# Iamctb/ImageStitching

Hardware: AMD Instinct MI355X
Metric: stitched megapixels/sec (9x12 MP vertical) (higher is better)
Workload: dtype u8

## Files before the change

### imagestitching_amd/csrc/ist_host.cpp

```cpp
#include "ist_host.h"

#include <algorithm>
#include <atomic>
#include <cstring>
#include <mutex>
#include <string>
#include <thread>

#include "ist_internal.h"

namespace ist {

namespace {

constexpr size_t kPoolGranule = 2u << 20;
constexpr size_t kPoolKeepBytes = 2ull << 30;
constexpr size_t kPoolKeepBlocks = 6;

constexpr size_t kPoolKeepBatchBytes = 8ull << 30;
constexpr size_t kPoolKeepBatchBlocks = 256;

struct Block { void* p; size_t cap; bool busy; uint64_t stamp; bool batch = false; };
std::mutex g_pool_mu;
std::vector<Block>& pool() { static std::vector<Block>* v = new std::vector<Block>(); return *v; }
uint64_t g_pool_clock = 0;

void pool_enforce_class_locked(bool batch) {
  const size_t keep_bytes = batch ? kPoolKeepBatchBytes : kPoolKeepBytes, keep_blocks = batch ? kPoolKeepBatchBlocks : kPoolKeepBlocks;
  for (;;) {
    size_t idle_bytes = 0, idle = 0, oldest = SIZE_MAX;
    std::vector<Block>& v = pool();
    for (size_t i = 0; i < v.size(); ++i) {
      if (v[i].busy || v[i].batch != batch) continue;
      idle_bytes += v[i].cap; ++idle;
      if (oldest == SIZE_MAX || v[i].stamp < v[oldest].stamp) oldest = i;
    }
    if (oldest == SIZE_MAX || (idle_bytes <= keep_bytes && idle <= keep_blocks)) return;
    (void)hipHostFree(v[oldest].p);
    v.erase(v.begin() + static_cast<std::ptrdiff_t>(oldest));
  }
}

void* pool_take_class(size_t bytes, bool batch) {
  const size_t need = ((bytes ? bytes : 1) + kPoolGranule - 1) / kPoolGranule * kPoolGranule;
  {
    std::lock_guard<std::mutex> lock(g_pool_mu);
    std::vector<Block>& v = pool();
    size_t best = SIZE_MAX;
    for (size_t i = 0; i < v.size(); ++i)
      if (!v[i].busy && v[i].batch == batch && v[i].cap >= need && v[i].cap <= 2 * need && (best == SIZE_MAX || v[i].cap < v[best].cap)) best = i;
    if (best != SIZE_MAX) { v[best].busy = true; v[best].stamp = ++g_pool_clock; return v[best].p; }
  }
  void* p = nullptr;
  if (hipHostMalloc(&p, need, hipHostMallocPortable) != hipSuccess) {
    (void)hipGetLastError();
    pool_trim();
    if (hipHostMalloc(&p, need, hipHostMallocPortable) != hipSuccess) { (void)hipGetLastError(); return nullptr; }
  }
  std::lock_guard<std::mutex> lock(g_pool_mu);
  pool().push_back(Block{p, need, true, ++g_pool_clock, batch});
  return p;
}

}

void* pool_take(size_t bytes) { return pool_take_class(bytes, false); }
void* pool_take_batch(size_t bytes) { return pool_take_class(bytes, true); }

bool pool_give(void* p) {
  std::lock_guard<std::mutex> lock(g_pool_mu);
  for (Block& b : pool())
    if (b.p == p) {
      b.busy = false; b.stamp = ++g_pool_clock;
      pool_enforce_class_locked(b.batch);
      return true;
    }
  return false;
}

void pool_trim() {
  std::lock_guard<std::mutex> lock(g_pool_mu);
  std::vector<Block>& v = pool();
  for (size_t i = v.size(); i-- > 0;)
    if (!v[i].busy) { (void)hipHostFree(v[i].p); v.erase(v.begin() + static_cast<std::ptrdiff_t>(i)); }
}

namespace {

constexpr size_t kChunk = 4u << 20;
constexpr int kLanes = 4;

struct Piece { uint32_t item; size_t row0, n_rows, col0, n_cols; };

void split(const std::vector<RowsCopy>& items, std::vector<Piece>* out) {
  for (size_t k = 0; k < items.size(); ++k) {
    const RowsCopy& it = items[k];
    if (it.row == 0 || it.rows == 0) continue;
    if (it.row <= kChunk) {
      const size_t per = kChunk / it.row;
      for (size_t r = 0; r < it.rows; r += per) out->push_back(Piece{static_cast<uint32_t>(k), r, std::min(per, it.rows - r), 0, it.row});
    } else {
      for (size_t r = 0; r < it.rows; ++r)
        for (size_t c = 0; c < it.row; c += kChunk) out->push_back(Piece{static_cast<uint32_t>(k), r, 1, c, std::min(kChunk, it.row - c)});
    }
  }
}

inline size_t piece_bytes(const Piece& p) { return p.n_rows * p.n_cols; }

void pack(const RowsCopy& it, const Piece& p, uint8_t* chunk) {
  const uint8_t* s = static_cast<const uint8_t*>(it.host_src) + p.row0 * it.host_pitch + p.col0;
  if (it.host_pitch == p.n_cols) { std::memcpy(chunk, s, p.n_rows * p.n_cols); return; }
  for (size_t r = 0; r < p.n_rows; ++r) std::memcpy(chunk + r * p.n_cols, s + r * it.host_pitch, p.n_cols);
}
void unpack(const RowsCopy& it, const Piece& p, const uint8_t* chunk) {
  uint8_t* d = static_cast<uint8_t*>(it.host_dst) + p.row0 * it.host_pitch + p.col0;
  if (it.host_pitch == p.n_cols) { std::memcpy(d, chunk, p.n_rows * p.n_cols); return; }
  for (size_t r = 0; r < p.n_rows; ++r) std::memcpy(d + r * it.host_pitch, chunk + r * p.n_cols, p.n_cols);
}
inline uint8_t* dev_of(const RowsCopy& it, const Piece& p) { return static_cast<uint8_t*>(it.dev) + p.row0 * it.row + p.col0; }

}

void Stager::release_lane(Lane& l) {
  if (l.stream) (void)hipStreamSynchronize(l.stream);
  for (int s = 0; s < 2; ++s) { if (l.done[s]) (void)hipEventDestroy(l.done[s]); if (l.chunk[s]) (void)hipHostFree(l.chunk[s]); l.done[s] = nullptr; l.chunk[s] = nullptr; }
  if (l.tail) (void)hipEventDestroy(l.tail);
  if (l.stream) (void)hipStreamDestroy(l.stream);
  l.tail = nullptr; l.stream = nullptr;
}

Stager::~Stager() {
  int prev = -1;
  (void)hipGetDevice(&prev);
  if (hipSetDevice(device_) != hipSuccess) return;
  if (big_.stream) (void)hipStreamSynchronize(big_.stream);
  for (int s = 0; s < 2; ++s) { if (big_.done[s]) (void)hipEventDestroy(big_.done[s]); if (big_.piece[s]) (void)hipHostFree(big_.piece[s]); }
  if (big_.tail) (void)hipEventDestroy(big_.tail);
  if (big_.stream) (void)hipStreamDestroy(big_.stream);
  for (Lane& l : lanes_) release_lane(l);
  if (gate_) (void)hipEventDestroy(gate_);
  if (prev >= 0) (void)hipSetDevice(prev);
}

int Stager::ensure() {
  if (!lanes_.empty()) return IST_OK;
  std::vector<Lane> lanes(kLanes);
  hipEvent_t gate = nullptr;
  bool ok = hipEventCreateWithFlags(&gate, hipEventDisableTiming) == hipSuccess;
  for (Lane& l : lanes) {
    ok = ok && hipStreamCreateWithFlags(&l.stream, hipStreamNonBlocking) == hipSuccess &&
         hipEventCreateWithFlags(&l.tail, hipEventDisableTiming) == hipSuccess;
    for (int s = 0; s < 2 && ok; ++s)
      ok = hipHostMalloc(&l.chunk[s], kChunk, hipHostMallocDefault) == hipSuccess &&
           hipEventCreateWithFlags(&l.done[s], hipEventDisableTiming) == hipSuccess &&
           hipEventRecord(l.done[s], l.stream) == hipSuccess;
  }
  if (!ok) {
    (void)hipGetLastError();
    for (Lane& l : lanes) release_lane(l);
    if (gate) (void)hipEventDestroy(gate);
    return fail(IST_E_HIP, "allocating the pinned staging ring failed");
  }
  lanes_.swap(lanes);
  gate_ = gate;
  return IST_OK;
}

namespace { constexpr size_t kBigPiece = 32u << 20; constexpr int kBigPackers = 4; }

int Stager::ensure_big() {
  if (big_.stream) return IST_OK;
  Big b;
  bool ok = hipStreamCreateWithFlags(&b.stream, hipStreamNonBlocking) == hipSuccess && hipEventCreateWithFlags(&b.tail, hipEventDisableTiming) == hipSuccess;
  for (int s = 0; s < 2 && ok; ++s)
    ok = hipHostMalloc(&b.piece[s], kBigPiece, hipHostMallocDefault) == hipSuccess && hipEventCreateWithFlags(&b.done[s], hipEventDisableTiming) == hipSuccess &&
         hipEventRecord(b.done[s], b.stream) == hipSuccess;
  if (!ok) {
    (void)hipGetLastError();
    for (int s = 0; s < 2; ++s) { if (b.done[s]) (void)hipEventDestroy(b.done[s]); if (b.piece[s]) (void)hipHostFree(b.piece[s]); }
    if (b.tail) (void)hipEventDestroy(b.tail);
    if (b.stream) (void)hipStreamDestroy(b.stream);
    return fail(IST_E_HIP, "allocating the large staging pieces failed");
  }
  big_ = b;
  return IST_OK;
}

int Stager::upload_big(const std::vector<RowsCopy>& items, hipStream_t after, WorkerPool* pool) {
  if (!pool) return upload(items, after);
  std::vector<RowsCopy> small;
  bool any = false;
  for (const RowsCopy& it : items) { if (it.row == 0 || it.rows == 0) continue; if (it.row > kBigPiece) small.push_back(it); else any = true; }
  if (!small.empty()) { const int rc = upload(small, after); if (rc) return rc; }
  if (!any) return IST_OK;
  int rc = ensure_big();
  if (rc) return rc;
  for (const RowsCopy& it : items) {
    if (it.row == 0 || it.rows == 0 || it.row > kBigPiece) continue;
    if (it.host_pitch == it.row) {
      hipPointerAttribute_t attr;
      std::memset(&attr, 0, sizeof(attr));
      if (hipPointerGetAttributes(&attr, it.host_src) == hipSuccess && attr.type == hipMemoryTypeHost) {
        if (hipMemcpyAsync(it.dev, it.host_src, it.rows * it.row, hipMemcpyHostToDevice, big_.stream) != hipSuccess) { (void)hipGetLastError(); return fail(IST_E_HIP, "host-to-device copy failed"); }
        continue;
      }
      (void)hipGetLastError();
    }
    const size_t per = std::max<size_t>(1, kBigPiece / it.row);
    for (size_t r0 = 0; r0 < it.rows; r0 += per) {
      const size_t nr = std::min(per, it.rows - r0);
      const int s = static_cast<int>(big_.k++ & 1u);
      if (hipEventSynchronize(big_.done[s]) != hipSuccess) { (void)hipGetLastError(); return fail(IST_E_HIP, "host-to-device staging failed"); }
      uint8_t* piece = static_cast<uint8_t*>(big_.piece[s]);
      const int workers = static_cast<int>(std::min<size_t>(kBigPackers, std::max<size_t>(1, nr * it.row >> 20)));
      const size_t share = (nr + static_cast<size_t>(workers) - 1) / static_cast<size_t>(workers);
      auto part = [&](int w) {
        const size_t a = static_cast<size_t>(w) * share, b = std::min(nr, a + share);
        if (a >= b) return;
        const uint8_t* src = static_cast<const uint8_t*>(it.host_src) + (r0 + a) * it.host_pitch;
        if (it.host_pitch == it.row) std::memcpy(piece + a * it.row, src, (b - a) * it.row);
        else for (size_t r = a; r < b; ++r) std::memcpy(piece + r * it.row, src + (r - a) * it.host_pitch, it.row);
      };
      if (workers > 1) { pool->run(workers, part); pool->wait(); } else part(0);
      if (hipMemcpyAsync(static_cast<uint8_t*>(it.dev) + r0 * it.row, piece, nr * it.row, hipMemcpyHostToDevice, big_.stream) != hipSuccess ||
          hipEventRecord(big_.done[s], big_.stream) != hipSuccess) { (void)hipGetLastError(); return fail(IST_E_HIP, "host-to-device staging failed"); }
    }
  }
  if (hipEventRecord(big_.tail, big_.stream) != hipSuccess || hipStreamWaitEvent(after, big_.tail, 0) != hipSuccess) { (void)hipGetLastError(); return fail(IST_E_HIP, "ordering the uploads before the launch failed"); }
  return IST_OK;
}

int Stager::sync() {
  bool ok = true;
  if (big_.stream) ok = hipStreamSynchronize(big_.stream) == hipSuccess;
  for (Lane& l : lanes_) if (l.stream) ok = (hipStreamSynchronize(l.stream) == hipSuccess) && ok;
  return ok ? IST_OK : fail(IST_E_HIP, "hipStreamSynchronize failed");
}

int Stager::upload(const std::vector<RowsCopy>& items, hipStream_t after) { return run(items, true, after); }
int Stager::download(const std::vector<RowsCopy>& items, hipStream_t before) { return run(items, false, before); }

int Stager::run(const std::vector<RowsCopy>& items, bool up, hipStream_t other) {
  std::vector<Piece> pieces;
  split(items, &pieces);
  if (pieces.empty()) return IST_OK;
  int rc = ensure();
  if (rc) return rc;
  size_t total = 0;
  for (const Piece& p : pieces) total += piece_bytes(p);
  const int n_lanes = total < (2u << 20) ? 1 : static_cast<int>(std::min<size_t>(kLanes, pieces.size()));
  if (!up) {
    if (hipEventRecord(gate_, other) != hipSuccess) return fail(IST_E_HIP, "hipEventRecord failed");
    for (int l = 0; l < n_lanes; ++l)
      if (hipStreamWaitEvent(lanes_[static_cast<size_t>(l)].stream, gate_, 0) != hipSuccess) return fail(IST_E_HIP, "hipStreamWaitEvent failed");
  }
  std::atomic<size_t> next{0};
  std::atomic<int> err{0};
  auto work = [&](int li) {
    if (hipSetDevice(device_) != hipSuccess) { err = 1; return; }
    Lane& L = lanes_[static_cast<size_t>(li)];
    const Piece* pending[2] = {nullptr, nullptr};
    unsigned k = 0;
    for (;;) {
      const size_t i = next.fetch_add(1);
      if (i >= pieces.size() || err.load()) break;
      const Piece& p = pieces[i];
      const RowsCopy& it = items[p.item];
      const int s = static_cast<int>(k++ & 1u);
      if (hipEventSynchronize(L.done[s]) != hipSuccess) { err = 1; break; }
      uint8_t* chunk = static_cast<uint8_t*>(L.chunk[s]);
      if (up) {
        pack(it, p, chunk);
        if (hipMemcpyAsync(dev_of(it, p), chunk, piece_bytes(p), hipMemcpyHostToDevice, L.stream) != hipSuccess) { err = 1; break; }
      } else {
        if (pending[s]) { unpack(items[pending[s]->item], *pending[s], chunk); pending[s] = nullptr; }
        if (hipMemcpyAsync(chunk, dev_of(it, p), piece_bytes(p), hipMemcpyDeviceToHost, L.stream) != hipSuccess) { err = 1; break; }
        pending[s] = &p;
      }
      if (hipEventRecord(L.done[s], L.stream) != hipSuccess) { err = 1; break; }
    }
    if (!up)
      for (unsigned d = 0; d < 2; ++d) {
        const int s = static_cast<int>((k + d) & 1u);
        if (!pending[s]) continue;
        if (hipEventSynchronize(L.done[s]) != hipSuccess) { err = 1; continue; }
        unpack(items[pending[s]->item], *pending[s], static_cast<const uint8_t*>(L.chunk[s]));
      }
  };
  if (n_lanes == 1) work(0);
  else {
    std::vector<std::thread> th;
    for (int l = 1; l < n_lanes; ++l) th.emplace_back(work, l);
    work(0);
    for (std::thread& t : th) t.join();
  }
  if (err.load()) { (void)hipGetLastError(); return fail(IST_E_HIP, up ? "host-to-device staging failed" : "device-to-host staging failed"); }
  if (up)
    for (int l = 0; l < n_lanes; ++l) {
      Lane& L = lanes_[static_cast<size_t>(l)];
      if (hipEventRecord(L.tail, L.stream) != hipSuccess || hipStreamWaitEvent(other, L.tail, 0) != hipSuccess)
        return fail(IST_E_HIP, "ordering the uploads before the launch failed");
    }
  return IST_OK;
}


WorkerPool::~WorkerPool() {
  { std::lock_guard<std::mutex> lock(mu_); stop_ = true; }
  work_cv_.notify_all();
  for (std::thread& t : th_) if (t.joinable()) t.join();
}

void WorkerPool::loop() {
  std::unique_lock<std::mutex> lock(mu_);
  for (;;) {
    work_cv_.wait(lock, [&]() { return stop_ || next_ < total_; });
    if (stop_) return;
    const int i = next_++;
    lock.unlock();
    fn_(i);
    lock.lock();
    if (++done_ == total_) done_cv_.notify_all();
  }
}

void WorkerPool::run(int n, std::function<void(int)> fn) {
  if (n <= 0) return;
  {
    std::lock_guard<std::mutex> lock(mu_);
    tl_mark("pool: queue locked");
    fn_ = std::move(fn);
    next_ = 0; done_ = 0; total_ = n;
    const size_t want = static_cast<size_t>(n < kMaxThreads ? n : kMaxThreads);
    while (th_.size() < want) th_.emplace_back([this]() { loop(); });
  }
  tl_mark("pool: tasks posted");
  work_cv_.notify_all();
  tl_mark("pool: workers notified");
}

void WorkerPool::wait() {
  std::unique_lock<std::mutex> lock(mu_);
  done_cv_.wait(lock, [&]() { return done_ == total_; });
  total_ = 0; next_ = 0; done_ = 0;
}

}
```

### imagestitching_amd/csrc/ist_host.h

```cpp
#ifndef IST_HOST_H_
#define IST_HOST_H_

#include <hip/hip_runtime_api.h>

#include <cstddef>
#include <thread>
#include <mutex>
#include <functional>
#include <condition_variable>
#include <cstdint>
#include <vector>

#include "ist_internal.h"

namespace ist {

void* pool_take(size_t bytes);
void* pool_take_batch(size_t bytes);
bool pool_give(void* p);
void pool_trim();

class Stager {
 public:
  explicit Stager(int device) : device_(device) {}
  ~Stager();
  Stager(const Stager&) = delete;
  Stager& operator=(const Stager&) = delete;
  int upload(const std::vector<RowsCopy>& items, hipStream_t after);
  int download(const std::vector<RowsCopy>& items, hipStream_t before);
  int sync();
  int upload_big(const std::vector<RowsCopy>& items, hipStream_t after, class WorkerPool* pool);

 private:
  struct Lane { hipStream_t stream = nullptr; void* chunk[2] = {nullptr, nullptr}; hipEvent_t done[2] = {nullptr, nullptr}; hipEvent_t tail = nullptr; };
  int ensure();
  static void release_lane(Lane& l);
  int run(const std::vector<RowsCopy>& items, bool up, hipStream_t other);
  int device_;
  std::vector<Lane> lanes_;
  hipEvent_t gate_ = nullptr;
  struct Big { hipStream_t stream = nullptr; void* piece[2] = {nullptr, nullptr}; hipEvent_t done[2] = {nullptr, nullptr}; hipEvent_t tail = nullptr; unsigned k = 0; } big_;
  int ensure_big();
};


class WorkerPool {
 public:
  static constexpr int kMaxThreads = 32;
  WorkerPool() = default;
  ~WorkerPool();
  WorkerPool(const WorkerPool&) = delete;
  WorkerPool& operator=(const WorkerPool&) = delete;
  void run(int n, std::function<void(int)> fn);
  void wait();
 private:
  void loop();
  std::mutex mu_;
  std::condition_variable work_cv_, done_cv_;
  std::vector<std::thread> th_;
  std::function<void(int)> fn_;
  int next_ = 0, total_ = 0, done_ = 0;
  bool stop_ = false;
};

}

#endif
```

### imagestitching_amd/csrc/ist_host_stitch.cpp

```cpp
#include <algorithm>
#include <atomic>
#include <chrono>
#include <cstdio>
#include <cstdlib>
#include <mutex>
#include <vector>

#include "ist_ctx.h"

using namespace ist;

namespace {

std::atomic<int64_t> g_duplex_stitches{0};

int render_to_scratch(ist_ctx* ctx, int64_t canvas_w, int64_t canvas_h, const uint8_t clear_rgba[4],
                      const ist_op* ops, int n_ops, const ist_image_desc* images, const uint8_t* const* src,
                      const size_t* src_pitch, int n_images, int filter, const ist_region* region,
                      int64_t* out_w, int64_t* out_h) {
  const JobPtr job(ist_job_create(ctx, canvas_w, canvas_h, clear_rgba, ops, n_ops, images, n_images, filter, region));
  if (!job) return g_last_code ? g_last_code : IST_E_INVALID;

  SourceLayout lay;
  int rc = lay.add(images, n_images, src, src_pitch, whole_bitmaps(job->host));
  if (rc) return rc;
  rc = grow_device(&ctx->scratch_src, &ctx->scratch_src_bytes, lay.bytes());
  if (rc) return rc;
  const int64_t rw = job->host.rx1 - job->host.rx0, rh = job->host.ry1 - job->host.ry0;
  const size_t pitch = static_cast<size_t>(rw) * 4;
  rc = grow_device(&ctx->scratch_dst, &ctx->scratch_dst_bytes, pitch * static_cast<size_t>(rh));
  if (rc) return rc;
  const SourceLayout::Placed at = lay.place(ctx->scratch_src);
  std::vector<RowsCopy> up;
  lay.copy_all(&up);
  rc = stager_of(ctx).upload(up, ctx->stream);
  if (rc) return rc;
  const uintptr_t biased = reinterpret_cast<uintptr_t>(ctx->scratch_dst) - (static_cast<uintptr_t>(job->host.ry0) * pitch + static_cast<uintptr_t>(job->host.rx0) * 4);
  rc = ist_job_launch(job.get(), at.ptr.data(), at.pitch.data(), n_images, reinterpret_cast<void*>(biased), pitch, ctx->stream);
  if (rc) return rc;
  IST_HIP(hipStreamSynchronize(ctx->stream));
  if (out_w) *out_w = rw;
  if (out_h) *out_h = rh;
  return IST_OK;
}

struct RowBands {
  ist_ctx* ctx = nullptr;
  bool ok = false;
  int nb = 0, n_images = 0;
  int64_t cw = 0, ch = 0;
  size_t row = 0, total = 0;
  const ist_image_desc* images = nullptr;
  std::vector<int32_t> cuts;
  std::vector<std::map<int, RowSpan>> need;
  std::vector<JobPtr> jobs;
  SourceLayout lay;
  SourceLayout::Placed at;
  std::vector<int64_t> lo, hi;
  std::vector<RowsCopy> items;
  uint8_t* canvas = nullptr;
  int64_t y0(int b) const { return cuts[static_cast<size_t>(b)]; }
  int64_t y1(int b) const { return cuts[static_cast<size_t>(b) + 1]; }

  int prepare(ist_ctx* c, int64_t canvas_w, int64_t canvas_h, const uint8_t clear[4], const ist_op* ops, int n_ops, const ist_image_desc* imgs,
              const uint8_t* const* s, const size_t* sp, int n, int filter) {
    static const bool off = tuning_mode() && std::getenv("IST_HOST_DUPLEX") && std::atoi(std::getenv("IST_HOST_DUPLEX")) == 0;
    ctx = c; cw = canvas_w; ch = canvas_h; images = imgs; n_images = n;
    row = static_cast<size_t>(cw) * 4; total = row * static_cast<size_t>(ch);
    if (off || total < (32u << 20) || n_images < 1) return IST_OK;
    nb = static_cast<int>(std::min<size_t>(16, std::max<size_t>(2, total / (40u << 20))));
    cuts.assign(static_cast<size_t>(nb) + 1, 0);
    std::vector<ist_part> parts(static_cast<size_t>(std::max(1, n_ops)) * static_cast<size_t>(nb) + 8);
    int n_parts = 0;
    {
      KeepLastError keep;
      if (ist_shard_row_cuts(ch, nb, cuts.data()) != IST_OK ||
          ist_shard_parts(ops, n_ops, cw, ch, images, n_images, filter, nb, IST_SPLIT_ROWS, parts.data(), static_cast<int>(parts.size()), &n_parts) != IST_OK)
        return IST_OK;
    }
    parts.resize(static_cast<size_t>(n_parts));
    jobs.resize(static_cast<size_t>(nb)); need.resize(static_cast<size_t>(nb));
    for (int b = 0; b < nb; ++b) {
      need[static_cast<size_t>(b)] = shard_holdings(parts_of_slot(parts, b));
      if (y0(b) >= y1(b)) continue;
      const ist_region clip{0, static_cast<int32_t>(y0(b)), static_cast<int32_t>(cw), static_cast<int32_t>(y1(b) - y0(b))};
      jobs[static_cast<size_t>(b)].reset(ist_job_create(ctx, cw, ch, clear, ops, n_ops, images, n_images, filter, &clip));
      if (!jobs[static_cast<size_t>(b)]) return g_last_code ? g_last_code : IST_E_INVALID;
    }
    std::map<int, RowSpan> whole;
    for (const auto& band : need) for (const auto& kv : band) whole[kv.first] = RowSpan{0, bitmap_h(images[kv.first])};
    int rc = lay.add(images, n_images, s, sp, whole);
    if (rc) return rc;
    rc = grow_device(&ctx->scratch_src, &ctx->scratch_src_bytes, lay.bytes());
    if (rc) return rc;
    rc = grow_device(&ctx->scratch_dst, &ctx->scratch_dst_bytes, total);
    if (rc) return rc;
    at = lay.place(ctx->scratch_src);
    lo.assign(static_cast<size_t>(n_images), -1); hi.assign(static_cast<size_t>(n_images), -1);
    canvas = static_cast<uint8_t*>(ctx->scratch_dst);
    ok = true;
    return IST_OK;
  }

  int submit(int b, hipStream_t R) {
    items.clear();
    auto send = [&](int i, int64_t r0, int64_t r1) { if (r1 > r0) items.push_back(lay.copy(i, r0, r1)); };
    for (const auto& kv : need[static_cast<size_t>(b)]) {
      const int i = kv.first;
      const int64_t a = std::max<int64_t>(0, kv.second.y0), e = std::min<int64_t>(bitmap_h(images[i]), kv.second.y1);
      if (e <= a) continue;
      int64_t& L0 = lo[static_cast<size_t>(i)]; int64_t& H0 = hi[static_cast<size_t>(i)];
      if (L0 < 0) { send(i, a, e); L0 = a; H0 = e; }
      else {
        if (a < L0) { send(i, a, L0); L0 = a; }
        if (e > H0) { send(i, H0, e); H0 = e; }
      }
    }
    if (!items.empty()) { const int rc = stager_of(ctx).upload_big(items, R, &workers_of(ctx)); if (rc) return rc; }
    return ist_job_launch(jobs[static_cast<size_t>(b)].get(), at.ptr.data(), at.pitch.data(), n_images, canvas, row, R);
  }
};

int stitch_banded_duplex(ist_ctx* ctx, const ist_plan* plan, const ist_op* ops, int n_ops, const ist_image_desc* images,
                         const uint8_t* const* src, const size_t* src_pitch, int n_images, int filter, uint8_t** out_pixels, bool* done) {
  *done = false;
  static const bool print = std::getenv("IST_TIMING") != nullptr;
  const auto t_start = std::chrono::steady_clock::now();
  auto lap = [&](const char* what) { if (print) std::fprintf(stderr, "[ist timing] host stitch: %-34s at %7.2f ms\n", what, std::chrono::duration<double, std::milli>(std::chrono::steady_clock::now() - t_start).count()); };
  RowBands rb;
  int rc = rb.prepare(ctx, plan->canvas_w, plan->canvas_h, kTransparent, ops, n_ops, images, src, src_pitch, n_images, filter);
  if (rc) return rc;
  if (!rb.ok) return IST_OK;
  rc = ensure_aux(ctx);
  if (rc) return rc;
  lap("band jobs compiled, scratch");
  uint8_t* host = static_cast<uint8_t*>(pool_take(rb.total));
  if (!host) return fail(IST_E_NOMEM, "out of pinned host memory for the result");
  std::vector<hipEvent_t> ev(static_cast<size_t>(rb.nb), nullptr);
  hipStream_t R = ctx->stream, D = ctx->aux;
  auto finish = [&](int code) {
    (void)hipStreamSynchronize(R); (void)hipStreamSynchronize(D); (void)stager_of(ctx).sync();
    for (hipEvent_t e : ev) if (e) (void)hipEventDestroy(e);
    if (code != IST_OK) pool_give(host);
    return code;
  };
  bool first = true;
  for (int b = 0; b < rb.nb; ++b) {
    const int64_t y0 = rb.y0(b), y1 = rb.y1(b);
    if (y0 >= y1) continue;
    rc = rb.submit(b, R);
    if (rc) return finish(rc);
    hipEvent_t& e = ev[static_cast<size_t>(b)];
    if (hipEventCreateWithFlags(&e, hipEventDisableTiming) != hipSuccess || hipEventRecord(e, R) != hipSuccess || hipStreamWaitEvent(D, e, 0) != hipSuccess ||
        hipMemcpyAsync(host + static_cast<size_t>(y0) * rb.row, rb.canvas + static_cast<size_t>(y0) * rb.row, static_cast<size_t>(y1 - y0) * rb.row, hipMemcpyDeviceToHost, D) != hipSuccess) {
      (void)hipGetLastError();
      return finish(fail(IST_E_HIP, "queueing a band's readback failed"));
    }
    if (first) { lap("first band queued"); first = false; }
  }
  lap("last band queued");
  if (hipStreamSynchronize(D) != hipSuccess || hipStreamSynchronize(R) != hipSuccess) { (void)hipGetLastError(); return finish(fail(IST_E_HIP, "result readback failed")); }
  lap("last band in host memory");
  g_duplex_stitches.fetch_add(1, std::memory_order_relaxed);
  *out_pixels = host;
  *done = true;
  return finish(IST_OK);
}

int render_png_banded(ist_ctx* ctx, int64_t canvas_w, int64_t canvas_h, const uint8_t clear_rgba[4], const ist_op* ops, int n_ops,
                      const ist_image_desc* images, const uint8_t* const* src, const size_t* src_pitch, int n_images, int filter,
                      uint8_t** out_png, int64_t* out_len, ist_preview* preview) {
  RowBands rb;
  int rc = rb.prepare(ctx, canvas_w, canvas_h, clear_rgba ? clear_rgba : kTransparent, ops, n_ops, images, src, src_pitch, n_images, filter);
  if (rc) return rc;
  if (!rb.ok) return 1;
  rc = ensure_render(ctx);
  if (rc) return rc;
  hipStream_t R = ctx->render;
  std::vector<hipEvent_t> ev(static_cast<size_t>(rb.nb), nullptr);
  int next = 0;
  auto need_rows = [&](int64_t y_end, void* reader_) -> int {
    hipStream_t reader = static_cast<hipStream_t>(reader_);
    int last = -1;
    for (int b = 0; b < rb.nb; ++b) {
      if (rb.y0(b) >= rb.y1(b)) continue;
      if (rb.y0(b) >= y_end) break;
      if (b >= next) {
        const int rc2 = rb.submit(b, R);
        if (rc2) return rc2;
        if (hipEventCreateWithFlags(&ev[static_cast<size_t>(b)], hipEventDisableTiming) != hipSuccess || hipEventRecord(ev[static_cast<size_t>(b)], R) != hipSuccess) {
          (void)hipGetLastError(); return fail(IST_E_HIP, "hipEventRecord failed");
        }
        next = b + 1;
      }
      last = b;
    }
    if (last >= 0 && hipStreamWaitEvent(reader, ev[static_cast<size_t>(last)], 0) != hipSuccess) { (void)hipGetLastError(); return fail(IST_E_HIP, "ordering the export behind the render failed"); }
    return IST_OK;
  };
  int64_t hint = 0;
  for (int b = 0; b < rb.nb; ++b) hint = std::max<int64_t>(hint, rb.y1(b) - rb.y0(b));
  rc = png_to_host(ctx, rb.canvas, rb.row, canvas_w, canvas_h, nullptr, out_png, out_len, need_rows, hint, preview);
  (void)hipStreamSynchronize(R); (void)stager_of(ctx).sync(); (void)hipStreamSynchronize(ctx->stream);
  for (hipEvent_t e : ev) if (e) (void)hipEventDestroy(e);
  if (rc == IST_OK) g_duplex_stitches.fetch_add(1, std::memory_order_relaxed);
  return rc;
}

int render_png(ist_ctx* ctx, int64_t canvas_w, int64_t canvas_h, const uint8_t clear_rgba[4], const ist_op* ops, int n_ops,
               const ist_image_desc* images, const uint8_t* const* src, const size_t* src_pitch, int n_images, int filter,
               uint8_t** out_png, int64_t* out_len, ist_preview* preview) {
  *out_png = nullptr; *out_len = 0;
  { const int rc = ctx_png_form_check(ctx); if (rc) return rc; }
  std::lock_guard<std::mutex> lock(ctx->mu);
  DeviceGuard g(ctx->device);
  int rc = render_png_banded(ctx, canvas_w, canvas_h, clear_rgba, ops, n_ops, images, src, src_pitch, n_images, filter, out_png, out_len, preview);
  if (rc != 1) return rc;
  rc = render_to_scratch(ctx, canvas_w, canvas_h, clear_rgba, ops, n_ops, images, src, src_pitch, n_images, filter, nullptr, nullptr, nullptr);
  if (rc) return rc;
  return png_to_host(ctx, ctx->scratch_dst, static_cast<size_t>(canvas_w) * 4, canvas_w, canvas_h, nullptr, out_png, out_len, nullptr, 0, preview);
}

}

extern "C" {

int64_t ist_debug_duplex_stitches(void) { return g_duplex_stitches.load(); }

int ist_render_rgba8(ist_ctx* ctx, int64_t canvas_w, int64_t canvas_h, const uint8_t clear_rgba[4],
                     const ist_op* ops, int n_ops, const ist_image_desc* images, const uint8_t* const* src,
                     const size_t* src_pitch, int n_images, int filter, const ist_region* region, uint8_t* dst,
                     size_t dst_pitch) {
  if (!ctx) return fail(IST_E_NO_CONTEXT, "无法获取绘图上下文");
  if (!dst) return fail(IST_E_INVALID, "ist_render_rgba8: dst is NULL");
  std::lock_guard<std::mutex> lock(ctx->mu);
  DeviceGuard g(ctx->device);
  int64_t rw = canvas_w, rh = canvas_h;
  if (region) {
    const int64_t rx = std::max<int64_t>(0, region->x), ry = std::max<int64_t>(0, region->y);
    rw = std::min<int64_t>(canvas_w, static_cast<int64_t>(region->x) + region->w) - rx;
    rh = std::min<int64_t>(canvas_h, static_cast<int64_t>(region->y) + region->h) - ry;
  }
  if (rw > 0 && dst_pitch < static_cast<size_t>(rw) * 4) return fail(IST_E_INVALID, "dst_pitch too small");
  int rc = render_to_scratch(ctx, canvas_w, canvas_h, clear_rgba, ops, n_ops, images, src, src_pitch, n_images, filter, region, &rw, &rh);
  if (rc) return rc;
  std::vector<RowsCopy> down{RowsCopy{ctx->scratch_dst, nullptr, dst, dst_pitch, static_cast<size_t>(rw) * 4, static_cast<size_t>(rh)}};
  return stager_of(ctx).download(down, ctx->stream);
}

int ist_render_png(ist_ctx* ctx, int64_t canvas_w, int64_t canvas_h, const uint8_t clear_rgba[4], const ist_op* ops,
                   int n_ops, const ist_image_desc* images, const uint8_t* const* src, const size_t* src_pitch,
                   int n_images, int filter, uint8_t** out_png, int64_t* out_len) {
  if (!ctx) return fail(IST_E_NO_CONTEXT, "无法获取绘图上下文");
  if (!out_png || !out_len) return fail(IST_E_INVALID, "ist_render_png: NULL output");
  return render_png(ctx, canvas_w, canvas_h, clear_rgba, ops, n_ops, images, src, src_pitch, n_images, filter, out_png, out_len, nullptr);
}

int ist_stitch_png_preview(ist_ctx* ctx, const ist_image_desc* images, const uint8_t* const* src, const size_t* src_pitch,
                           int n_images, int direction, int mode, double gap, const ist_limits* limits, int filter,
                           ist_plan* out_plan, uint8_t** out_png, int64_t* out_len, ist_preview* preview) {
  preview_clear(preview);
  if (!ctx) return fail(IST_E_NO_CONTEXT, "无法获取绘图上下文");
  if (!out_plan || !out_png || !out_len) return fail(IST_E_INVALID, "ist_stitch_png: NULL output");
  int rc = preview_check(preview);
  if (rc) return rc;
  std::vector<ist_op> ops;
  rc = plan_with_ops(images, n_images, direction, mode, gap, limits, out_plan, &ops);
  if (rc != IST_OK) return rc;
  rc = render_png(ctx, out_plan->canvas_w, out_plan->canvas_h, kTransparent, ops.data(), static_cast<int>(ops.size()), images, src, src_pitch,
                  n_images, filter, out_png, out_len, preview);
  if (rc != IST_OK) ist_plan_free(out_plan);
  return rc;
}

int ist_stitch_png(ist_ctx* ctx, const ist_image_desc* images, const uint8_t* const* src, const size_t* src_pitch,
                   int n_images, int direction, int mode, double gap, const ist_limits* limits, int filter,
                   ist_plan* out_plan, uint8_t** out_png, int64_t* out_len) {
  return ist_stitch_png_preview(ctx, images, src, src_pitch, n_images, direction, mode, gap, limits, filter, out_plan, out_png, out_len, nullptr);
}

int ist_stitch_rgba8(ist_ctx* ctx, const ist_image_desc* images, const uint8_t* const* src, const size_t* src_pitch,
                     int n_images, int direction, int mode, double gap, const ist_limits* limits, int filter,
                     ist_plan* out_plan, uint8_t** out_pixels) {
  if (!ctx) return fail(IST_E_NO_CONTEXT, "无法获取绘图上下文");
  if (!out_plan || !out_pixels) return fail(IST_E_INVALID, "ist_stitch_rgba8: NULL output");
  *out_pixels = nullptr;
  std::vector<ist_op> ops;
  int rc = plan_with_ops(images, n_images, direction, mode, gap, limits, out_plan, &ops);
  if (rc != IST_OK) return rc;
  PlanGuard pg{out_plan};
  const int n_ops = static_cast<int>(ops.size());
  {
    std::lock_guard<std::mutex> lock(ctx->mu);
    DeviceGuard g(ctx->device);
    bool done = false;
    rc = stitch_banded_duplex(ctx, out_plan, ops.data(), n_ops, images, src, src_pitch, n_images, filter, out_pixels, &done);
    if (rc == IST_OK && !done) {
      rc = render_to_scratch(ctx, out_plan->canvas_w, out_plan->canvas_h, kTransparent, ops.data(), n_ops, images, src, src_pitch,
                             n_images, filter, nullptr, nullptr, nullptr);
      if (rc == IST_OK)
        rc = read_back_pooled(ctx->scratch_dst, static_cast<size_t>(out_plan->canvas_w) * 4 * static_cast<size_t>(out_plan->canvas_h), ctx->stream, out_pixels);
    }
  }
  pg.keep = rc == IST_OK;
  return rc;
}

int ist_stitch_jpeg(ist_ctx* ctx, const ist_image_desc* images, const uint8_t* const* src, const size_t* src_pitch,
                    int n_images, int direction, int mode, double gap, const ist_limits* limits, int filter, int quality,
                    int subsampling, ist_plan* out_plan, uint8_t** out_jpeg, int64_t* out_len) {
  if (!ctx) return fail(IST_E_NO_CONTEXT, "无法获取绘图上下文");
  if (!out_plan || !out_jpeg || !out_len) return fail(IST_E_INVALID, "ist_stitch_jpeg: NULL output");
  *out_jpeg = nullptr; *out_len = 0;
  int rc = jpeg_check_options("ist_stitch_jpeg", quality, subsampling);
  if (rc) return rc;
// ... 35 lines not shown
```

Measured before the change: 811,500.

## Plan banded uploads up front and pack multiple items into shared staging pieces

Host-to-device uploads for the banded stitch are now planned once for all bands. Small items are packed together into shared 32 MiB pinned pieces, and the first piece is shortened to 8 MiB so the first band's kernel can start sooner. Each band then sends only the pieces it needs before launching. Packer threads rise from 4 to 8 (capped by the CPU budget), the last two pieces are rebalanced, and optional streaming stores, a 3-deep ring and timing instrumentation sit behind env knobs. This aims to cut per-item copy and sync overhead and to overlap packing with transfer and compute, at the cost of more complex bookkeeping.

```diff
diff --git a/imagestitching_amd/csrc/ist_host.cpp b/imagestitching_amd/csrc/ist_host.cpp
--- a/imagestitching_amd/csrc/ist_host.cpp
+++ b/imagestitching_amd/csrc/ist_host.cpp
@@ -2,12 +2,19 @@
 
 #include <algorithm>
 #include <atomic>
+#include <chrono>
+#include <cstdio>
+#include <cstdlib>
 #include <cstring>
 #include <mutex>
 #include <string>
 #include <thread>
+#if defined(__linux__)
+#include <sched.h>
+#endif
 
 #include "ist_internal.h"
+#include "ist_pack.h"
 
 namespace ist {
 
@@ -134,10 +141,7 @@
   int prev = -1;
   (void)hipGetDevice(&prev);
   if (hipSetDevice(device_) != hipSuccess) return;
-  if (big_.stream) (void)hipStreamSynchronize(big_.stream);
-  for (int s = 0; s < 2; ++s) { if (big_.done[s]) (void)hipEventDestroy(big_.done[s]); if (big_.piece[s]) (void)hipHostFree(big_.piece[s]); }
-  if (big_.tail) (void)hipEventDestroy(big_.tail);
-  if (big_.stream) (void)hipStreamDestroy(big_.stream);
+  release_big(big_);
   for (Lane& l : lanes_) release_lane(l);
   if (gate_) (void)hipEventDestroy(gate_);
   if (prev >= 0) (void)hipSetDevice(prev);
@@ -167,69 +171,189 @@
   return IST_OK;
 }
 
-namespace { constexpr size_t kBigPiece = 32u << 20; constexpr int kBigPackers = 4; }
+namespace {
+
+constexpr size_t kBigPiece = 32u << 20;
+constexpr size_t kFirstPiece = 8u << 20;
+constexpr int kBigPackers = 8;
+constexpr int kBigRing = 2;
+
+using Clock = std::chrono::steady_clock;
+inline double ms_since(Clock::time_point t) { return std::chrono::duration<double, std::milli>(Clock::now() - t).count(); }
+bool big_timing() { static const bool on = std::getenv("IST_TIMING") != nullptr; return on; }
+long knob(const char* name, long dflt) {
+  const char* e = tuning_mode() ? std::getenv(name) : nullptr;
+  return e && *e ? std::atol(e) : dflt;
+}
+
+int cpu_budget() {
+  int n = static_cast<int>(std::thread::hardware_concurrency());
+#if defined(__linux__)
+  cpu_set_t set;
+  CPU_ZERO(&set);
+  if (sched_getaffinity(0, sizeof(set), &set) == 0 && CPU_COUNT(&set) > 0) n = CPU_COUNT(&set);
+  if (std::FILE* f = std::fopen("/sys/fs/cgroup/cpu.max", "r")) {
+    char quota[32] = {0};
+    long period = 0;
+    if (std::fscanf(f, "%31s %ld", quota, &period) == 2 && period > 0 && std::strcmp(quota, "max") != 0) {
+      const long q = (std::atol(quota) + period - 1) / period;
+      if (q > 0 && q < n) n = static_cast<int>(q);
+    }
+    std::fclose(f);
+  }
+#endif
+  return n > 0 ? n : 1;
+}
+int packer_cap() { static const int cap = std::max(2, std::min(cpu_budget(), 16) - 1); return cap; }
+int big_packers() { static const int n = static_cast<int>(std::max<long>(1, std::min<long>(packer_cap(), knob("IST_PACKERS", kBigPackers)))); return n; }
+int big_ring() { static const int n = static_cast<int>(std::max<long>(2, std::min<long>(3, knob("IST_BIG_RING", kBigRing)))); return n; }
+size_t first_piece() { static const size_t n = static_cast<size_t>(std::max<long>(1, std::min<long>(32, knob("IST_FIRST_PIECE_MIB", static_cast<long>(kFirstPiece >> 20))))) << 20; return n; }
+PackBody pack_body() { static const PackBody b = knob("IST_PACK_STREAM", 0) ? kPackStream : kPackMemcpy; return b; }
+
+}
+
+void Stager::release_big(Big& b) {
+  if (b.stream) (void)hipStreamSynchronize(b.stream);
+  for (int s = 0; s < kMaxRing; ++s) { if (b.done[s]) (void)hipEventDestroy(b.done[s]); if (b.piece[s]) (void)hipHostFree(b.piece[s]); }
+  if (b.tail) (void)hipEventDestroy(b.tail);
+  if (b.stream) (void)hipStreamDestroy(b.stream);
+  b = Big();
+}
 
 int Stager::ensure_big() {
   if (big_.stream) return IST_OK;
   Big b;
+  b.ring = big_ring();
   bool ok = hipStreamCreateWithFlags(&b.stream, hipStreamNonBlocking) == hipSuccess && hipEventCreateWithFlags(&b.tail, hipEventDisableTiming) == hipSuccess;
-  for (int s = 0; s < 2 && ok; ++s)
+  for (int s = 0; s < b.ring && ok; ++s)
     ok = hipHostMalloc(&b.piece[s], kBigPiece, hipHostMallocDefault) == hipSuccess && hipEventCreateWithFlags(&b.done[s], hipEventDisableTiming) == hipSuccess &&
          hipEventRecord(b.done[s], b.stream) == hipSuccess;
   if (!ok) {
     (void)hipGetLastError();
-    for (int s = 0; s < 2; ++s) { if (b.done[s]) (void)hipEventDestroy(b.done[s]); if (b.piece[s]) (void)hipHostFree(b.piece[s]); }
-    if (b.tail) (void)hipEventDestroy(b.tail);
-    if (b.stream) (void)hipStreamDestroy(b.stream);
+    release_big(b);
     return fail(IST_E_HIP, "allocating the large staging pieces failed");
   }
   big_ = b;
+  return IST_OK;
+}
+
+int Stager::plan(std::vector<UploadItem> items, int n_bands, bool short_first_piece, Planned* out) {
+  for (UploadItem& it : items) {
+    it.staged = it.rows != 0 && it.row != 0 && it.row <= kBigPiece;
+    if (it.staged && it.host_pitch == it.row) {
+      hipPointerAttribute_t attr;
+      std::memset(&attr, 0, sizeof(attr));
+      if (hipPointerGetAttributes(&attr, it.host_src) == hipSuccess && attr.type == hipMemoryTypeHost) it.staged = false;
+      else (void)hipGetLastError();
+    }
+  }
+  out->plan = plan_upload(items, n_bands, kBigPiece, short_first_piece ? first_piece() : kBigPiece);
+  out->items = std::move(items);
+  out->next_item = 0; out->next_piece = 0;
+  return IST_OK;
+}
+
+int Stager::send_piece(const Planned& p, int q, WorkerPool* pool) {
+  const UploadPiece& pc = p.plan.pieces[static_cast<size_t>(q)];
+  const bool timed = big_timing();
+  const int s = static_cast<int>(big_.k++ % static_cast<unsigned>(big_.ring));
+  Clock::time_point t0 = Clock::now();
+  if (hipEventSynchronize(big_.done[s]) != hipSuccess) { (void)hipGetLastError(); return fail(IST_E_HIP, "host-to-device staging failed"); }
+  if (timed) timing_.sync_ms += ms_since(t0);
+  uint8_t* piece = static_cast<uint8_t*>(big_.piece[s]);
+  std::vector<PackFragment> frags(pc.n);
+  for (size_t k = 0; k < pc.n; ++k) {
+    const UploadFragment& f = p.plan.frags[pc.first + k];
+    const UploadItem& it = p.items[f.item];
+    frags[k] = PackFragment{static_cast<const uint8_t*>(it.host_src) + f.row0 * it.host_pitch, it.host_pitch, it.row, f.rows, f.at};
+  }
+  const PackBody body = pack_body();
+  const int workers = static_cast<int>(std::min<size_t>(static_cast<size_t>(big_packers()), std::max<size_t>(1, pc.bytes >> 20)));
+  std::atomic<int64_t> busiest{0};
+  auto part = [&](int w) {
+    const Clock::time_point w0 = timed ? Clock::now() : Clock::time_point();
+    size_t a, b;
+    pack_slice_bounds(pc.bytes, workers, w, &a, &b);
+    if (a < b) pack_slice(piece, frags.data(), frags.size(), a, b, body);
+    if (timed) {
+      const int64_t ns = std::chrono::duration_cast<std::chrono::nanoseconds>(Clock::now() - w0).count();
+      int64_t seen = busiest.load();
+      while (ns > seen && !busiest.compare_exchange_weak(seen, ns)) {}
+    }
+  };
+  t0 = Clock::now();
+  if (workers > 1) { pool->run(workers, part); pool->wait(); } else part(0);
+  if (timed) {
+    const double wall = ms_since(t0), pack = static_cast<double>(busiest.load()) * 1e-6;
+    timing_.pack_ms += pack; timing_.pool_ms += std::max(0.0, wall - pack);
+    ++timing_.pieces; timing_.sizes.push_back(pc.bytes);
+  }
+  t0 = Clock::now();
+  for (size_t k = 0; k < pc.n; ++k) {
+    const UploadFragment& f = p.plan.frags[pc.first + k];
+    const UploadItem& it = p.items[f.item];
+    if (hipMemcpyAsync(static_cast<uint8_t*>(it.dev) + f.row0 * it.row, piece + f.at, f.rows * it.row, hipMemcpyHostToDevice, big_.stream) != hipSuccess) {
+      (void)hipGetLastError();
+      (void)hipEventRecord(big_.done[s], big_.stream);
+      return fail(IST_E_HIP, "host-to-device staging failed");
+    }
+  }
+  if (hipEventRecord(big_.done[s], big_.stream) != hipSuccess) { (void)hipGetLastError(); return fail(IST_E_HIP, "host-to-device staging failed"); }
+  if (timed) timing_.submit_ms += ms_since(t0);
+  return IST_OK;
+}
+
+int Stager::send_through(Planned* p, int band, hipStream_t after, WorkerPool* pool) {
+  if (band < 0 || static_cast<size_t>(band) >= p->plan.last_piece.size()) return fail(IST_E_INVALID, "upload plan: no such band");
+  std::vector<RowsCopy> chunked;
+  bool direct = false;
+  for (; p->next_item < p->items.size() && p->items[p->next_item].band <= band; ++p->next_item) {
+    const UploadItem& it = p->items[p->next_item];
+    if (it.staged || it.rows == 0 || it.row == 0) continue;
+    if (it.row > kBigPiece) { chunked.push_back(RowsCopy{it.dev, it.host_src, nullptr, it.host_pitch, it.row, it.rows}); continue; }
+    int rc = ensure_big();
+    if (rc) return rc;
+    if (hipMemcpyAsync(it.dev, it.host_src, it.rows * it.row, hipMemcpyHostToDevice, big_.stream) != hipSuccess) { (void)hipGetLastError(); return fail(IST_E_HIP, "host-to-device copy failed"); }
+    direct = true;
+  }
+  if (!chunked.empty()) { const int rc = upload(chunked, after); if (rc) return rc; }
+  const int last = p->plan.last_piece[static_cast<size_t>(band)];
+  bool sent = false;
+  for (; p->next_piece <= last; ++p->next_piece) {
+    int rc = ensure_big();
+    if (rc == IST_OK) rc = send_piece(*p, p->next_piece, pool);
+    if (rc) return rc;
+    sent = true;
+  }
+  if (!big_.stream || (!sent && !direct && last < 0)) return IST_OK;
+  hipEvent_t ev = big_.done[(big_.k + static_cast<unsigned>(big_.ring) - 1) % static_cast<unsigned>(big_.ring)];
+  if (direct || big_.k == 0) {
+    if (hipEventRecord(big_.tail, big_.stream) != hipSuccess) { (void)hipGetLastError(); return fail(IST_E_HIP, "ordering the uploads before the launch failed"); }
+    ev = big_.tail;
+  }
+  if (hipStreamWaitEvent(after, ev, 0) != hipSuccess) { (void)hipGetLastError(); return fail(IST_E_HIP, "ordering the uploads before the launch failed"); }
   return IST_OK;
 }
 
 int Stager::upload_big(const std::vector<RowsCopy>& items, hipStream_t after, WorkerPool* pool) {
   if (!pool) return upload(items, after);
-  std::vector<RowsCopy> small;
-  bool any = false;
-  for (const RowsCopy& it : items) { if (it.row == 0 || it.rows == 0) continue; if (it.row > kBigPiece) small.push_back(it); else any = true; }
-  if (!small.empty()) { const int rc = upload(small, after); if (rc) return rc; }
-  if (!any) return IST_OK;
-  int rc = ensure_big();
-  if (rc) return rc;
-  for (const RowsCopy& it : items) {
-    if (it.row == 0 || it.rows == 0 || it.row > kBigPiece) continue;
-    if (it.host_pitch == it.row) {
-      hipPointerAttribute_t attr;
-      std::memset(&attr, 0, sizeof(attr));
-      if (hipPointerGetAttributes(&attr, it.host_src) == hipSuccess && attr.type == hipMemoryTypeHost) {
-        if (hipMemcpyAsync(it.dev, it.host_src, it.rows * it.row, hipMemcpyHostToDevice, big_.stream) != hipSuccess) { (void)hipGetLastError(); return fail(IST_E_HIP, "host-to-device copy failed"); }
-        continue;
-      }
-      (void)hipGetLastError();
-    }
-    const size_t per = std::max<size_t>(1, kBigPiece / it.row);
-    for (size_t r0 = 0; r0 < it.rows; r0 += per) {
-      const size_t nr = std::min(per, it.rows - r0);
-      const int s = static_cast<int>(big_.k++ & 1u);
-      if (hipEventSynchronize(big_.done[s]) != hipSuccess) { (void)hipGetLastError(); return fail(IST_E_HIP, "host-to-device staging failed"); }
-      uint8_t* piece = static_cast<uint8_t*>(big_.piece[s]);
-      const int workers = static_cast<int>(std::min<size_t>(kBigPackers, std::max<size_t>(1, nr * it.row >> 20)));
-      const size_t share = (nr + static_cast<size_t>(workers) - 1) / static_cast<size_t>(workers);
-      auto part = [&](int w) {
-        const size_t a = static_cast<size_t>(w) * share, b = std::min(nr, a + share);
-        if (a >= b) return;
-        const uint8_t* src = static_cast<const uint8_t*>(it.host_src) + (r0 + a) * it.host_pitch;
-        if (it.host_pitch == it.row) std::memcpy(piece + a * it.row, src, (b - a) * it.row);
-        else for (size_t r = a; r < b; ++r) std::memcpy(piece + r * it.row, src + (r - a) * it.host_pitch, it.row);
-      };
-      if (workers > 1) { pool->run(workers, part); pool->wait(); } else part(0);
-      if (hipMemcpyAsync(static_cast<uint8_t*>(it.dev) + r0 * it.row, piece, nr * it.row, hipMemcpyHostToDevice, big_.stream) != hipSuccess ||
-          hipEventRecord(big_.done[s], big_.stream) != hipSuccess) { (void)hipGetLastError(); return fail(IST_E_HIP, "host-to-device staging failed"); }
-    }
-  }
-  if (hipEventRecord(big_.tail, big_.stream) != hipSuccess || hipStreamWaitEvent(after, big_.tail, 0) != hipSuccess) { (void)hipGetLastError(); return fail(IST_E_HIP, "ordering the uploads before the launch failed"); }
-  return IST_OK;
-}
+  std::vector<UploadItem> list;
+  list.reserve(items.size());
+  for (const RowsCopy& it : items) list.push_back(UploadItem{static_cast<int>(list.size()), 0, it.rows, it.row, it.host_pitch, it.host_src, it.dev, 0, false});
+  Planned p;
+  const int rc = plan(std::move(list), 1, false, &p);
+  return rc ? rc : send_through(&p, 0, after, pool);
+}
+
+void Stager::timing_begin() { timing_ = BigTiming(); }
+void Stager::timing_report(const char* what) {
+  if (!big_timing()) return;
+  std::string sizes;
+  for (size_t b : timing_.sizes) { char t[32]; std::snprintf(t, sizeof(t), " %.1f", static_cast<double>(b) / (1u << 20)); sizes += t; }
+  std::fprintf(stderr, "[ist timing] %s: big pieces %d (MiB:%s); packing %.2f ms, blocked on a staging piece's event %.2f ms, pool run/wait overhead %.2f ms, queueing the copies %.2f ms; packers %d, ring %d\n",
+               what, timing_.pieces, sizes.c_str(), timing_.pack_ms, timing_.sync_ms, timing_.pool_ms, timing_.submit_ms, big_packers(), big_.ring);
+}
+
 
 int Stager::sync() {
   bool ok = true;
diff --git a/imagestitching_amd/csrc/ist_host.h b/imagestitching_amd/csrc/ist_host.h
--- a/imagestitching_amd/csrc/ist_host.h
+++ b/imagestitching_amd/csrc/ist_host.h
@@ -12,6 +12,7 @@
 #include <vector>
 
 #include "ist_internal.h"
+#include "ist_upload_plan.h"
 
 namespace ist {
 
@@ -30,6 +31,11 @@
   int download(const std::vector<RowsCopy>& items, hipStream_t before);
   int sync();
   int upload_big(const std::vector<RowsCopy>& items, hipStream_t after, class WorkerPool* pool);
+  struct Planned { std::vector<UploadItem> items; UploadPlan plan; size_t next_item = 0; int next_piece = 0; };
+  int plan(std::vector<UploadItem> items, int n_bands, bool short_first_piece, Planned* out);
+  int send_through(Planned* p, int band, hipStream_t after, class WorkerPool* pool);
+  void timing_begin();
+  void timing_report(const char* what);
 
  private:
   struct Lane { hipStream_t stream = nullptr; void* chunk[2] = {nullptr, nullptr}; hipEvent_t done[2] = {nullptr, nullptr}; hipEvent_t tail = nullptr; };
@@ -39,8 +45,12 @@
   int device_;
   std::vector<Lane> lanes_;
   hipEvent_t gate_ = nullptr;
-  struct Big { hipStream_t stream = nullptr; void* piece[2] = {nullptr, nullptr}; hipEvent_t done[2] = {nullptr, nullptr}; hipEvent_t tail = nullptr; unsigned k = 0; } big_;
+  static constexpr int kMaxRing = 3;
+  struct Big { hipStream_t stream = nullptr; int ring = 0; void* piece[kMaxRing] = {}; hipEvent_t done[kMaxRing] = {}; hipEvent_t tail = nullptr; unsigned k = 0; } big_;
   int ensure_big();
+  static void release_big(Big& b);
+  int send_piece(const Planned& p, int q, class WorkerPool* pool);
+  struct BigTiming { int pieces = 0; double pack_ms = 0, sync_ms = 0, pool_ms = 0, submit_ms = 0; std::vector<size_t> sizes; } timing_;
 };
 
 
diff --git a/imagestitching_amd/csrc/ist_host_stitch.cpp b/imagestitching_amd/csrc/ist_host_stitch.cpp
--- a/imagestitching_amd/csrc/ist_host_stitch.cpp
+++ b/imagestitching_amd/csrc/ist_host_stitch.cpp
@@ -56,8 +56,7 @@
   std::vector<JobPtr> jobs;
   SourceLayout lay;
   SourceLayout::Placed at;
-  std::vector<int64_t> lo, hi;
-  std::vector<RowsCopy> items;
+  Stager::Planned up;
   uint8_t* canvas = nullptr;
   int64_t y0(int b) const { return cuts[static_cast<size_t>(b)]; }
   int64_t y1(int b) const { return cuts[static_cast<size_t>(b) + 1]; }
@@ -69,6 +68,8 @@
     row = static_cast<size_t>(cw) * 4; total = row * static_cast<size_t>(ch);
     if (off || total < (32u << 20) || n_images < 1) return IST_OK;
     nb = static_cast<int>(std::min<size_t>(16, std::max<size_t>(2, total / (40u << 20))));
+    static const int nb_knob = (tuning_mode() && std::getenv("IST_HOST_BANDS")) ? std::atoi(std::getenv("IST_HOST_BANDS")) : 0;
+    if (nb_knob >= 2 && nb_knob <= 16) nb = nb_knob;
     cuts.assign(static_cast<size_t>(nb) + 1, 0);
     std::vector<ist_part> parts(static_cast<size_t>(std::max(1, n_ops)) * static_cast<size_t>(nb) + 8);
     int n_parts = 0;
@@ -96,27 +97,37 @@
     rc = grow_device(&ctx->scratch_dst, &ctx->scratch_dst_bytes, total);
     if (rc) return rc;
     at = lay.place(ctx->scratch_src);
-    lo.assign(static_cast<size_t>(n_images), -1); hi.assign(static_cast<size_t>(n_images), -1);
     canvas = static_cast<uint8_t*>(ctx->scratch_dst);
+    std::vector<int64_t> lo(static_cast<size_t>(n_images), -1), hi(static_cast<size_t>(n_images), -1);
+    std::vector<UploadItem> items;
+    for (int b = 0; b < nb; ++b) {
+      if (y0(b) >= y1(b)) continue;
+      auto send = [&](int i, int64_t r0, int64_t r1) {
+        if (r1 <= r0) return;
+        const RowsCopy c = lay.copy(i, r0, r1);
+        items.push_back(UploadItem{i, r0, c.rows, c.row, c.host_pitch, c.host_src, c.dev, b, false});
+      };
+      for (const auto& kv : need[static_cast<size_t>(b)]) {
+        const int i = kv.first;
+        const int64_t a = std::max<int64_t>(0, kv.second.y0), e = std::min<int64_t>(bitmap_h(images[i]), kv.second.y1);
+        if (e <= a) continue;
+        int64_t& L0 = lo[static_cast<size_t>(i)]; int64_t& H0 = hi[static_cast<size_t>(i)];
+        if (L0 < 0) { send(i, a, e); L0 = a; H0 = e; }
+        else {
+          if (a < L0) { send(i, a, L0); L0 = a; }
+          if (e > H0) { send(i, H0, e); H0 = e; }
+        }
+      }
+    }
+    rc = stager_of(ctx).plan(std::move(items), nb, true, &up);
+    if (rc) return rc;
     ok = true;
     return IST_OK;
   }
 
   int submit(int b, hipStream_t R) {
-    items.clear();
-    auto send = [&](int i, int64_t r0, int64_t r1) { if (r1 > r0) items.push_back(lay.copy(i, r0, r1)); };
-    for (const auto& kv : need[static_cast<size_t>(b)]) {
-      const int i = kv.first;
-      const int64_t a = std::max<int64_t>(0, kv.second.y0), e = std::min<int64_t>(bitmap_h(images[i]), kv.second.y1);
-      if (e <= a) continue;
-      int64_t& L0 = lo[static_cast<size_t>(i)]; int64_t& H0 = hi[static_cast<size_t>(i)];
-      if (L0 < 0) { send(i, a, e); L0 = a; H0 = e; }
-      else {
-        if (a < L0) { send(i, a, L0); L0 = a; }
-        if (e > H0) { send(i, H0, e); H0 = e; }
-      }
-    }
-    if (!items.empty()) { const int rc = stager_of(ctx).upload_big(items, R, &workers_of(ctx)); if (rc) return rc; }
+    const int rc = stager_of(ctx).send_through(&up, b, R, &workers_of(ctx));
+    if (rc) return rc;
     return ist_job_launch(jobs[static_cast<size_t>(b)].get(), at.ptr.data(), at.pitch.data(), n_images, canvas, row, R);
   }
 };
@@ -128,6 +139,7 @@
   const auto t_start = std::chrono::steady_clock::now();
   auto lap = [&](const char* what) { if (print) std::fprintf(stderr, "[ist timing] host stitch: %-34s at %7.2f ms\n", what, std::chrono::duration<double, std::milli>(std::chrono::steady_clock::now() - t_start).count()); };
   RowBands rb;
+  if (print) stager_of(ctx).timing_begin();
   int rc = rb.prepare(ctx, plan->canvas_w, plan->canvas_h, kTransparent, ops, n_ops, images, src, src_pitch, n_images, filter);
   if (rc) return rc;
   if (!rb.ok) return IST_OK;
@@ -161,6 +173,7 @@
   lap("last band queued");
   if (hipStreamSynchronize(D) != hipSuccess || hipStreamSynchronize(R) != hipSuccess) { (void)hipGetLastError(); return finish(fail(IST_E_HIP, "result readback failed")); }
   lap("last band in host memory");
+  if (print) stager_of(ctx).timing_report("host stitch");
   g_duplex_stitches.fetch_add(1, std::memory_order_relaxed);
   *out_pixels = host;
   *done = true;
diff --git a/imagestitching_amd/csrc/ist_pack.h b/imagestitching_amd/csrc/ist_pack.h
--- /dev/null
+++ b/imagestitching_amd/csrc/ist_pack.h
@@ -0,0 +1,79 @@
+#ifndef IST_PACK_H_
+#define IST_PACK_H_
+
+#include <cstddef>
+#include <cstdint>
+#include <cstring>
+
+#if defined(__SSE2__)
+#include <emmintrin.h>
+#endif
+
+namespace ist {
+
+enum PackBody { kPackMemcpy = 0, kPackStream = 1 };
+
+inline void pack_bytes(uint8_t* dst, const uint8_t* src, size_t n, PackBody body) {
+#if defined(__SSE2__)
+  if (body == kPackStream && n >= 256) {
+    const size_t head = (16 - (reinterpret_cast<uintptr_t>(dst) & 15)) & 15;
+    std::memcpy(dst, src, head);
+    dst += head; src += head; n -= head;
+    size_t i = 0;
+    for (; i + 64 <= n; i += 64) {
+      const __m128i a = _mm_loadu_si128(reinterpret_cast<const __m128i*>(src + i)), b = _mm_loadu_si128(reinterpret_cast<const __m128i*>(src + i + 16));
+      const __m128i c = _mm_loadu_si128(reinterpret_cast<const __m128i*>(src + i + 32)), d = _mm_loadu_si128(reinterpret_cast<const __m128i*>(src + i + 48));
+      _mm_stream_si128(reinterpret_cast<__m128i*>(dst + i), a); _mm_stream_si128(reinterpret_cast<__m128i*>(dst + i + 16), b);
+      _mm_stream_si128(reinterpret_cast<__m128i*>(dst + i + 32), c); _mm_stream_si128(reinterpret_cast<__m128i*>(dst + i + 48), d);
+    }
+    std::memcpy(dst + i, src + i, n - i);
+    return;
+  }
+#endif
+  (void)body;
+  std::memcpy(dst, src, n);
+}
+inline void pack_fence(PackBody body) {
+#if defined(__SSE2__)
+  if (body == kPackStream) _mm_sfence();
+#endif
+  (void)body;
+}
+
+inline void pack_rows(uint8_t* dst, const uint8_t* src, size_t host_pitch, size_t row_bytes, size_t rows, PackBody body = kPackMemcpy) {
+  if (host_pitch == row_bytes) { pack_bytes(dst, src, rows * row_bytes, body); return; }
+  for (size_t r = 0; r < rows; ++r) pack_bytes(dst + r * row_bytes, src + r * host_pitch, row_bytes, body);
+}
+
+struct PackFragment { const uint8_t* src; size_t host_pitch, row, rows, at; };
+
+inline void pack_slice_bounds(size_t bytes, int n_workers, int w, size_t* a, size_t* b) {
+  const size_t n = n_workers > 0 ? static_cast<size_t>(n_workers) : 1;
+  const size_t per = ((bytes + n - 1) / n + 63) / 64 * 64;
+  *a = per * static_cast<size_t>(w) < bytes ? per * static_cast<size_t>(w) : bytes;
+  *b = bytes - *a < per ? bytes : *a + per;
+}
+
+inline void pack_slice(uint8_t* piece, const PackFragment* f, size_t n, size_t a, size_t b, PackBody body = kPackMemcpy) {
+  for (size_t k = 0; k < n; ++k) {
+    const PackFragment& g = f[k];
+    const size_t len = g.row * g.rows;
+    if (len == 0 || g.at >= b || g.at + len <= a) continue;
+    size_t lo = a > g.at ? a - g.at : 0;
+    const size_t hi = b - g.at < len ? b - g.at : len;
+    uint8_t* dst = piece + g.at;
+    if (lo % g.row) {
+      const size_t r = lo / g.row, c = lo % g.row, m = hi - lo < g.row - c ? hi - lo : g.row - c;
+      pack_bytes(dst + lo, g.src + r * g.host_pitch + c, m, body);
+      lo += m;
+    }
+    const size_t whole = (hi - lo) / g.row;
+    if (whole) { pack_rows(dst + lo, g.src + lo / g.row * g.host_pitch, g.host_pitch, g.row, whole, body); lo += whole * g.row; }
+    if (lo < hi) pack_bytes(dst + lo, g.src + lo / g.row * g.host_pitch, hi - lo, body);
+  }
+  pack_fence(body);
+}
+
+}
+
+#endif
diff --git a/imagestitching_amd/csrc/ist_upload_plan.h b/imagestitching_amd/csrc/ist_upload_plan.h
--- /dev/null
+++ b/imagestitching_amd/csrc/ist_upload_plan.h
@@ -0,0 +1,97 @@
+#ifndef IST_UPLOAD_PLAN_H_
+#define IST_UPLOAD_PLAN_H_
+
+#include <cstddef>
+#include <cstdint>
+#include <vector>
+
+namespace ist {
+
+struct UploadItem {
+  int image; int64_t row0;
+  size_t rows, row, host_pitch;
+  const void* host_src;
+  void* dev;
+  int band;
+  bool staged;
+};
+struct UploadFragment { uint32_t item; size_t row0, rows, at; };
+struct UploadPiece { size_t first, n, bytes; };
+struct UploadPlan {
+  std::vector<UploadFragment> frags;
+  std::vector<UploadPiece> pieces;
+  std::vector<int> last_piece;
+};
+
+inline UploadPlan plan_upload(const std::vector<UploadItem>& items, int n_bands, size_t cap, size_t first_cap) {
+  UploadPlan p;
+  p.last_piece.assign(static_cast<size_t>(n_bands > 0 ? n_bands : 0), -1);
+  if (first_cap > cap || first_cap == 0) first_cap = cap;
+  struct Run { uint32_t item; size_t row0, rows, row; };
+  auto cut = [&](const std::vector<Run>& runs, size_t first_piece_cap, std::vector<std::vector<Run>>* out) {
+    std::vector<Run> cur; size_t used = 0, room = first_piece_cap;
+    for (const Run& r : runs) {
+      size_t r0 = r.row0, left = r.rows;
+      while (left) {
+        size_t fit = (room - used) / r.row;
+        if (fit == 0) { if (!cur.empty()) out->push_back(cur); cur.clear(); used = 0; room = cap; fit = room / r.row; }
+        const size_t take = fit < left ? fit : left;
+        cur.push_back(Run{r.item, r0, take, r.row});
+        used += take * r.row; r0 += take; left -= take;
+      }
+    }
+    if (!cur.empty()) out->push_back(cur);
+  };
+  std::vector<Run> stream;
+  for (size_t k = 0; k < items.size(); ++k) {
+    const UploadItem& it = items[k];
+    if (!it.staged || it.rows == 0 || it.row == 0 || it.row > cap) continue;
+    stream.push_back(Run{static_cast<uint32_t>(k), 0, it.rows, it.row});
+  }
+  std::vector<std::vector<Run>> pieces;
+  cut(stream, first_cap, &pieces);
+  auto bytes_of = [](const std::vector<Run>& v) { size_t b = 0; for (const Run& r : v) b += r.rows * r.row; return b; };
+  const size_t np = pieces.size();
+  if (np >= 2 && !(np == 2 && first_cap < cap) && bytes_of(pieces[np - 1]) < cap / 2) {
+    std::vector<Run> both = pieces[np - 2];
+    both.insert(both.end(), pieces[np - 1].begin(), pieces[np - 1].end());
+    const size_t half = (bytes_of(both) + 1) / 2;
+    std::vector<Run> a, b; size_t used = 0;
+    bool a_open = true;
+    for (const Run& r : both) {
+      size_t to_a = 0;
+      if (a_open) {
+        to_a = (half - used + r.row - 1) / r.row;
+        if (to_a > r.rows) to_a = r.rows;
+        if (to_a > (cap - used) / r.row) to_a = (cap - used) / r.row;
+        used += to_a * r.row;
+        if (to_a < r.rows || used >= half) a_open = false;
+      }
+      if (to_a) a.push_back(Run{r.item, r.row0, to_a, r.row});
+      if (to_a < r.rows) b.push_back(Run{r.item, r.row0 + to_a, r.rows - to_a, r.row});
+    }
+    if (!a.empty() && !b.empty() && bytes_of(b) <= cap) { pieces[np - 2] = a; pieces[np - 1] = b; }
+  }
+  std::vector<int> piece_of_item(items.size(), -1);
+  for (size_t q = 0; q < pieces.size(); ++q) {
+    UploadPiece pc{p.frags.size(), 0, 0};
+    for (const Run& r : pieces[q]) {
+      if (pc.n && p.frags.back().item == r.item && p.frags.back().row0 + p.frags.back().rows == r.row0) p.frags.back().rows += r.rows;
+      else { p.frags.push_back(UploadFragment{r.item, r.row0, r.rows, pc.bytes}); ++pc.n; }
+      pc.bytes += r.rows * r.row;
+      piece_of_item[r.item] = static_cast<int>(q);
+    }
+    p.pieces.push_back(pc);
+  }
+  int last = -1;
+  size_t k = 0;
+  for (int b = 0; b < n_bands; ++b) {
+    for (; k < items.size() && items[k].band <= b; ++k) if (piece_of_item[k] > last) last = piece_of_item[k];
+    p.last_piece[static_cast<size_t>(b)] = last;
+  }
+  return p;
+}
+
+}
+
+#endif
```

New measurement: 808,600. Within noise of the previous version (-0.4%).
